# nep-pack/NonlinearEigenproblems.jl

Measured on AMD Instinct MI355X. Metric: eigenpairs/sec (gun SPMF iar m=100) + compute_Mlincomb GB/s, higher is better.
Workload: dtype f64 (complex128)

## Files before the change

nonlineareigenproblems.jl_amd/csrc/common.h:

```cpp
#pragma once
#include <hip/hip_runtime.h>
#include <stdint.h>
#include <stdio.h>
#include <stdlib.h>
#include <string.h>
#include <stdarg.h>
#include "nepmi355.h"

typedef double2 cplx;

void nep_set_error(const char* fmt, ...);

#define HIPCHK(call)                                                                       \
    do {                                                                                   \
        hipError_t e_ = (call);                                                            \
        if (e_ != hipSuccess) {                                                            \
            nep_set_error("%s:%d: %s failed: %s", __FILE__, __LINE__, #call,               \
                          hipGetErrorString(e_));                                          \
            return NEP_ERR_HIP;                                                            \
        }                                                                                  \
    } while (0)

#define ARGCHK(cond)                                                                       \
    do {                                                                                   \
// ... 104 lines not shown
extern "C" {
int nep_cw_resid_dev(nep_spmf* s, const double* d_cabs, const nep_cdouble* d_ccf, const nep_cdouble* dx, const nep_cdouble* db,
                     nep_cdouble* dr, unsigned long long* d_bits, double xsign, hipStream_t st);
int nep_mlincomb_dev_shift(nep_spmf* s, int32_t k, const nep_cdouble* dC, int64_t ldc, const nep_cdouble* dV, int64_t ldv,
                           nep_cdouble* dz, nep_cdouble* d_shift, int32_t* folded, hipStream_t st);
int32_t nep_orth_dev_mirror(const nep_cdouble* dV, int64_t ldv, int64_t rows, int32_t k, const int64_t* d_active_rows,
                            nep_cdouble* dw, nep_cdouble* d_out, int32_t method, nep_cdouble* d_mirror, int32_t nmirror,
                            nep_stream stream);
int32_t nep_orth_dev_mirror_ev(const nep_cdouble* dV, int64_t ldv, int64_t rows, int32_t k, const int64_t* d_active_rows,
                               nep_cdouble* dw, nep_cdouble* d_out, int32_t method, nep_cdouble* d_mirror, int32_t nmirror,
                               void* before_write, nep_stream stream);
int32_t nep_orth_dev_iar_next(const nep_cdouble* dV, int64_t ldv, int64_t n, int32_t k, const int64_t* d_active_rows,
                              nep_cdouble* dw, nep_cdouble* d_out, int32_t method, nep_cdouble* d_mirror, int32_t nmirror,
                              void* before_write, const nep_cdouble* dC, int64_t ldc, int32_t mt, nep_cdouble* d_WT,
                              nep_cdouble* d_shift, nep_stream stream);
int nep_spmv_wt(nep_spmf* s, const nep_cdouble* d_WT, nep_cdouble* dz, hipStream_t st);
}

struct NepTiles;
extern "C" {
int nep_tiles_build(int64_t n, int mt, int valbytes, const int32_t* rowptr, const uint32_t* idx, const void* vals, NepTiles** out);
void nep_tiles_destroy(NepTiles* t);
void nep_tiles_info(const NepTiles* t, int64_t info[8]);
size_t nep_tiles_shmem(const NepTiles* t, int k);
int nep_tiles_mlincomb(const NepTiles* t, int k, const cplx* dC, int64_t ldc, const cplx* dV, int64_t ldv, cplx* dz, cplx* d_shift,
                       hipStream_t st);
int nep_tiles_nblk(const NepTiles* t);
bool nep_tiles_resid_ok(const NepTiles* t, int k);
bool nep_tiles_resid_cm_ok(const NepTiles* t, int k);
int nep_tiles_resid_cm(const NepTiles* t, int k, const cplx* dF, const cplx* Q, int64_t ldq, cplx* R, int64_t ldr, double* partial,
// ... 21 lines not shown
```

nonlineareigenproblems.jl_amd/csrc/driver.hip:

```cpp
#include "common.h"
#include <vector>
#include <stdlib.h>
#include <time.h>

struct nep_iar {
    nep_spmf* spmf; nep_lu* lu;
    int64_t n, ldv; int32_t m, mt;
    cplx* dV; const cplx* dCtab; int64_t ldc; const int64_t* d_active;
    cplx* dz; cplx* dW;
    std::vector<double> cabs; std::vector<nep_cdouble> cf;
    cplx* dH; nep_cdouble* hH;
    double* d_cabs; cplx* d_ccf;
    cplx* hH_dev;
    int32_t method;
    std::vector<hipEvent_t> ev;
    hipStream_t side = nullptr; hipEvent_t e_solved = nullptr, e_checked = nullptr;
    hipEvent_t e_upload = nullptr; bool upload_waited = false;
    hipStream_t last = nullptr;
    bool no_events = false;
    std::vector<hipGraphExec_t> graphs;
    cplx* dWT = nullptr; int32_t wt_for = 0;
};

extern "C" {

int32_t nep_iar_create(nep_spmf* spmf, nep_lu* lu, int64_t n, int32_t m, nep_cdouble* dV, int64_t ldv,
                       const nep_cdouble* dCtab, int64_t ldc, const int64_t* d_active, nep_cdouble* dwork3n,
                       const double* h_cabs, const nep_cdouble* h_cf, int32_t mt, nep_cdouble* dH, nep_cdouble* h_pinnedH,
                       int32_t orth_method, nep_iar** out) {
    ARGCHK(out != nullptr);
    *out = nullptr;
    ARGCHK(spmf && lu && dV && dCtab && dwork3n && dH && h_pinnedH);
    ARGCHK(n > 0 && m >= 1 && ldv >= n * (int64_t)(m + 1) && ldc >= m && mt >= 1 && (orth_method == 0 || orth_method == 1));
    nep_iar* s = new nep_iar();
    s->spmf = spmf; s->lu = lu; s->n = n; s->ldv = ldv; s->m = m; s->mt = mt;
    s->dV = (cplx*)dV; s->dCtab = (const cplx*)dCtab; s->ldc = ldc; s->d_active = d_active;
    s->dz = (cplx*)dwork3n; s->dW = (cplx*)dwork3n + n;
// ... 29 lines not shown
        void* dp = nullptr;
        if (hipHostGetDevicePointer(&dp, h_pinnedH, 0) == hipSuccess) s->hH_dev = (cplx*)dp; else (void)hipGetLastError();
    }
    *out = s;
    return NEP_OK;
}

int32_t nep_iar_destroy(nep_iar* s) {
    if (!s) return NEP_OK;
    for (hipEvent_t e : s->ev) if (e) (void)hipEventDestroy(e);
    if (!s->graphs.empty()) {
        if (s->last) (void)hipStreamSynchronize(s->last);
        for (hipGraphExec_t g : s->graphs) (void)hipGraphExecDestroy(g);
    }
    if (s->side) { (void)hipStreamSynchronize(s->side); (void)hipStreamDestroy(s->side); }
    if (s->e_solved) (void)hipEventDestroy(s->e_solved);
    if (s->e_checked) (void)hipEventDestroy(s->e_checked);
    if (s->e_upload) (void)hipEventDestroy(s->e_upload);
    if (s->d_cabs) nep_pool_free_on(s->d_cabs, s->last, s->last != nullptr);
    if (s->dWT) nep_pool_free_on(s->dWT, s->last, s->last != nullptr);
    delete s;
    return NEP_OK;
}

int32_t nep_iar_step(nep_iar* s, int32_t k, int32_t refine_steps, nep_stream stream) {
    const bool skip_final = (refine_steps & 0x100) != 0 && (k % 8) != 0;
    refine_steps &= 0xff;
    ARGCHK(s && k >= 1 && k <= s->m && refine_steps >= 0 && refine_steps <= 3);
    ARGCHK(refine_steps == 0 || !s->cabs.empty());
    hipStream_t st = as_stream(stream);
    const int64_t n = s->n;
    s->last = st;
    if (s->e_upload && !s->upload_waited) { HIPCHK(hipStreamWaitEvent(st, s->e_upload, 0)); s->upload_waited = true; }
    cplx* col = s->dV + (int64_t)(k - 1) * s->ldv;
    cplx* vv = s->dV + (int64_t)k * s->ldv;
    int32_t shifted = 0;
    int rc;
    if (s->dWT && s->wt_for == k) {
        rc = nep_spmv_wt(s->spmf, (const nep_cdouble*)s->dWT, (nep_cdouble*)s->dz, st);
        shifted = 1;
    } else
        rc = nep_mlincomb_dev_shift(s->spmf, k, (const nep_cdouble*)s->dCtab, s->ldc, (const nep_cdouble*)col, n, (nep_cdouble*)s->dz,
                                    (nep_cdouble*)(vv + n), &shifted, st);
    s->wt_for = 0;
    if (rc) return rc;
    cplx* hrow = s->dH + (int64_t)(k - 1) * (s->m + 4);
    unsigned long long* bits = (unsigned long long*)(hrow + k + 2);
    const bool record = !s->cabs.empty();
    if (refine_steps == 0) {
        rc = nep_lu_solve(s->lu, 1, (const nep_cdouble*)s->dz, n, (nep_cdouble*)vv, n, -1.0, stream);
        if (rc) return rc;
    } else {
// ... 16 lines not shown
        if (s->side) {
            HIPCHK(hipEventRecord(s->e_solved, st));
            HIPCHK(hipStreamWaitEvent(s->side, s->e_solved, 0));
            cs = s->side;
        }
        rc = nep_cw_resid_dev(s->spmf, s->d_cabs, (const nep_cdouble*)s->d_ccf, (const nep_cdouble*)vv, (const nep_cdouble*)s->dz,
                              (nep_cdouble*)s->dW, bits + refine_steps, -1.0, cs);
        if (rc) return rc;
        if (s->side) { HIPCHK(hipEventRecord(s->e_checked, s->side)); before_write = (void*)s->e_checked; }
    }
    if (!shifted) {
        rc = nep_iar_shift_scale(n, k, (const nep_cdouble*)col, (nep_cdouble*)vv, stream);
        if (rc) return rc;
    }
    cplx* mirror = s->hH_dev ? s->hH_dev + (int64_t)(k - 1) * (s->m + 4) : nullptr;
    if (s->dWT && k < s->m) {
        rc = nep_orth_dev_iar_next((const nep_cdouble*)s->dV, s->ldv, n, k, s->d_active, (nep_cdouble*)vv, (nep_cdouble*)hrow, s->method,
                                   (nep_cdouble*)mirror, k + 4, before_write, (const nep_cdouble*)s->dCtab, s->ldc, s->mt,
                                   (nep_cdouble*)s->dWT, (nep_cdouble*)(vv + s->ldv + n), stream);
        if (!rc) s->wt_for = k + 1;
    } else
        rc = nep_orth_dev_mirror_ev((const nep_cdouble*)s->dV, s->ldv, n * (int64_t)(k + 1), k, s->d_active, (nep_cdouble*)vv,
                                    (nep_cdouble*)hrow, s->method, (nep_cdouble*)mirror, k + 4, before_write, stream);
    if (rc) return rc;
    if (!mirror)
        HIPCHK(hipMemcpyAsync(s->hH + (int64_t)(k - 1) * (s->m + 4), hrow, (size_t)(k + 4) * sizeof(cplx), hipMemcpyDeviceToHost, st));
    if (s->no_events) return NEP_OK;
    if (!s->ev[k]) HIPCHK(hipEventCreateWithFlags(&s->ev[k], hipEventDisableTiming | hipEventBlockingSync));
    HIPCHK(hipEventRecord(s->ev[k], st));
    return NEP_OK;
}
// ... 67 lines not shown
```

nonlineareigenproblems.jl_amd/csrc/iar_run.hip:

```cpp
#include "common.h"
#include <algorithm>
#include <deque>
#include <map>
#include <mutex>
#include <vector>
#include <math.h>
#include <time.h>

extern "C" {
int32_t nep_iar_create(nep_spmf* spmf, nep_lu* lu, int64_t n, int32_t m, nep_cdouble* dV, int64_t ldv, const nep_cdouble* dCtab,
                       int64_t ldc, const int64_t* d_active, nep_cdouble* dwork3n, const double* h_cabs, const nep_cdouble* h_cf,
                       int32_t mt, nep_cdouble* dH, nep_cdouble* h_pinnedH, int32_t orth_method, nep_iar** out);
int32_t nep_iar_steps_graph(nep_iar* s, int32_t k0, int32_t count, int32_t refine_steps, nep_stream stream, int32_t* captured);
}

namespace {

constexpr double EPS = 2.220446049250313e-16;

__global__ void k_iar_active(int64_t* act, int64_t n, int m1) {
    const int j = blockIdx.x * blockDim.x + threadIdx.x;
    if (j < m1) act[j] = (int64_t)(j + 1) * n;
}
__global__ void k_iar_start(cplx* __restrict__ V, const cplx* __restrict__ v, double inv, int64_t n) {
    const int64_t i = (int64_t)blockIdx.x * blockDim.x + threadIdx.x;
    if (i < n) V[i] = cmake(v[i].x * inv, v[i].y * inv);
}

constexpr int64_t ZSLACK = 8192;
__global__ __launch_bounds__(256) void k_iar_zero_slack(cplx* __restrict__ V, int64_t ldv, int64_t n, int m1) {
    const int j = blockIdx.y;
    const int64_t a = (int64_t)(j + 1) * n;
    const int64_t r = a + (int64_t)blockIdx.x * 256 + threadIdx.x;
    if (j < m1 && r < ldv && r < a + ZSLACK) V[(int64_t)j * ldv + r] = cmake(0.0, 0.0);
}

struct RunStreams { hipStream_t check = nullptr, eig = nullptr; hipStream_t probed_for = (hipStream_t)-1; bool shared = false; int retries = 0; };
std::mutex g_rs_mu;
std::map<int, RunStreams> g_rs;

int pick_stream(hipStream_t keep, int prio, int ncand, bool probe, const std::vector<hipStream_t>& others, hipStream_t* out, bool* shared) {
    std::vector<hipStream_t> cand;
    if (keep) cand.push_back(keep);
    hipStream_t pick = nullptr;
    for (int c = 0; c < ncand && !pick; ++c) {
        hipStream_t s = nullptr;
        if ((size_t)c < cand.size()) s = cand[c];
        else { HIPCHK(hipStreamCreateWithPriority(&s, hipStreamNonBlocking, prio)); cand.push_back(s); }
        bool clash = false;
        for (size_t i = 0; probe && i < others.size() && !clash; ++i) {
            int32_t a = 0;
            int rc = nep_stream_pair_serializes((nep_stream)others[i], (nep_stream)s, &a); if (rc) return rc;
            clash = a != 0;
        }
        if (!clash) pick = s;
    }
    if (getenv("NEP_IAR_RUN_TRACE")) fprintf(stderr, "nep_iar_run: stream pick (prio %d): %zu candidates tried, %s\n", prio, cand.size(), pick ? "free queue found" : "none free");
    if (!pick) { pick = cand[0]; *shared = true; }
    for (hipStream_t s : cand) if (s != pick) (void)hipStreamDestroy(s);
    *out = pick;
    return NEP_OK;
}

int run_streams(hipStream_t main, RunStreams* out) {
    int dev = 0; HIPCHK(hipGetDevice(&dev));
    std::lock_guard<std::mutex> lk(g_rs_mu);
    RunStreams& r = g_rs[dev];
    if (!r.check || !r.eig || r.probed_for != main || (r.shared && r.retries < 3)) {
        if (r.shared) ++r.retries;
        r.shared = false;
        int least = 0, greatest = 0;
        HIPCHK(hipDeviceGetStreamPriorityRange(&least, &greatest));
        const int ncand = getenv("NEP_IAR_EIG_CANDIDATES") ? atoi(getenv("NEP_IAR_EIG_CANDIDATES")) : 8;
        const bool probe = !(getenv("NEP_IAR_EIG_PROBE") && atoi(getenv("NEP_IAR_EIG_PROBE")) == 0);
        const int cprio = getenv("NEP_IAR_CHECK_PRIO") ? (atoi(getenv("NEP_IAR_CHECK_PRIO")) > 0 ? least : (atoi(getenv("NEP_IAR_CHECK_PRIO")) < 0 ? greatest : 0)) : 0;
        int rc = pick_stream(r.check, cprio, ncand, probe, {main}, &r.check, &r.shared); if (rc) return rc;
        const int eprio = getenv("NEP_IAR_EIG_PRIO") ? (atoi(getenv("NEP_IAR_EIG_PRIO")) < 0 ? greatest : (atoi(getenv("NEP_IAR_EIG_PRIO")) > 0 ? least : 0)) : 0;
        rc = pick_stream(r.eig, eprio, ncand, probe, {main, r.check}, &r.eig, &r.shared); if (rc) return rc;
        r.probed_for = main;
    }
    *out = r;
    return NEP_OK;
}

struct Arena {
    int dev = -1; int64_t n = 0; int32_t m = 0, mt = 0;
    cplx* Hdev = nullptr; cplx* wdev = nullptr; cplx* Ctab = nullptr; cplx* work3n = nullptr; int64_t* active = nullptr;
    cplx* v0 = nullptr; double* d_norms = nullptr; void* eigwork = nullptr; int64_t wsz = 0; int bmax = 0;
    cplx* Hpin = nullptr; cplx* wpin = nullptr; double* npin = nullptr; cplx* stage = nullptr;
    void release() {
        for (void* p : {(void*)Hdev, (void*)wdev, (void*)Ctab, (void*)work3n, (void*)active, (void*)v0, (void*)d_norms, eigwork})
            if (p) nep_pool_free(p);
        for (void* p : {(void*)Hpin, (void*)wpin, (void*)npin, (void*)stage}) if (p) (void)hipHostFree(p);
        *this = Arena();
    }
};
std::mutex g_arena_mu;
std::vector<Arena> g_arenas;
// ... 143 lines not shown
};

}

extern "C" {

int32_t nep_refine_review(int32_t umfpack_refinements, int32_t plan, int32_t final_recorded, const double* w4, int32_t hint_in,
                          int32_t out[4]) {
    ARGCHK(w4 && out && plan >= 0 && plan <= 3 && umfpack_refinements >= 0);
    Refine r; r.umf = umfpack_refinements; r.hint = hint_in;
    const bool ok = r.review(w4, plan, final_recorded != 0);
    out[0] = ok ? 1 : 0; out[1] = r.recorded; out[2] = r.hint; out[3] = r.hint_off ? 1 : 0;
    return NEP_OK;
}

int32_t nep_iar_run(nep_spmf* spmf, nep_lu* lu, int64_t n, const nep_iar_opts* opts, const nep_cdouble* h_v0,
                    const nep_cdouble* h_Ctab, int32_t mt, const double* h_cabs, const nep_cdouble* h_cf, const double* h_fro,
                    nep_fv_eval fv, void* ctx, nep_cdouble* h_lam, nep_cdouble* dQ, nep_cdouble* h_Q, double* h_err,
                    nep_cdouble* dV_basis, nep_iar_result* res, nep_stream stream) {
    ARGCHK(spmf && lu && opts && h_v0 && h_Ctab && fv && h_lam && res);
    ARGCHK(n > 0 && mt >= 1 && opts->maxit >= 1 && opts->check_error_every >= 1);
    ARGCHK(opts->orth_method == 0 || opts->orth_method == 1);
    ARGCHK(opts->errmeasure == 0 || (opts->errmeasure == 1 && h_fro));
    ARGCHK(opts->umfpack_refinements <= 0 || (h_cabs && h_cf));
    memset(res, 0, sizeof(*res));
    res->refine_plan = -1;
    struct timespec t_e_; clock_gettime(CLOCK_MONOTONIC, &t_e_);
    const double t_entry = t_e_.tv_sec * 1e3 + t_e_.tv_nsec * 1e-6;
    const int32_t m = opts->maxit;
    if (m > 128) { nep_set_error("nep_iar_run: maxit = %d exceeds the device eigen-decomposition's limit 128", m); return NEP_ERR_UNSUPPORTED; }
    const int BMAX = std::max(1, getenv("NEP_IAR_EIG_BATCH") ? atoi(getenv("NEP_IAR_EIG_BATCH")) : 16);
    const int LASTB = std::max(1, getenv("NEP_IAR_EIG_LAST") ? atoi(getenv("NEP_IAR_EIG_LAST")) : 8);
    const double T100 = getenv("NEP_IAR_EIG_MS100") ? atof(getenv("NEP_IAR_EIG_MS100")) : 3.3;
    const double TSTEP = getenv("NEP_IAR_EIG_MSSTEP") ? atof(getenv("NEP_IAR_EIG_MSSTEP")) : 0.35;
    const int cee = opts->check_error_every;
    const double neigs = opts->neigs;
    const bool unthrottled = isinf(neigs) && neigs > 0;

    Run R; R.spmf = spmf; R.lu = lu; R.n = n; R.o = *opts; R.fv = fv; R.ctx = ctx; R.h_fro = h_fro; R.st = as_stream(stream);
    R.m = m; R.mt = mt; R.ldv = n * (int64_t)(m + 1); R.h_err = h_err;
    int rc = run_streams(R.st, &R.rs); if (rc) return rc;
    rc = arena_acquire(n, m, mt, BMAX, &R.a); if (rc) return rc;
    R.have_arena = true;
    Arena& a = R.a;
    hipStream_t st = R.st, cst = R.rs.check, est = R.rs.eig;
    R.ref.umf = opts->umfpack_refinements > 0 ? opts->umfpack_refinements : 0;
    R.ref.hint = (opts->refine_hint >= 0 && !(getenv("NEP_REFINE_HINT") && atoi(getenv("NEP_REFINE_HINT")) == 0)) ? opts->refine_hint : -1;
    R.filled.assign(m + 1, 0); R.plans.assign(m + 1, 0);
    if (const char* fa = getenv("NEP_IAR_RUN_FAIL_AT")) { if (sscanf(fa, "%d:%d", &R.fail_kind, &R.fail_at) != 2) R.fail_kind = R.fail_at = 0; }
    if (h_err) for (int64_t i = 0; i < (int64_t)m * m; ++i) h_err[i] = NAN;

    if (dV_basis) { R.V = (cplx*)dV_basis; R.own_V = false; }
    else {
        void* p = nullptr;
        rc = nep_pool_alloc(&p, (size_t)(m + 1) * R.ldv * 16); if (rc) return rc;
        R.V = (cplx*)p;
// ... 10 lines not shown
    }
    hipLaunchKernelGGL(k_iar_start, dim3((unsigned)((n + 255) / 256)), dim3(256), 0, st, R.V, (const cplx*)a.v0, 1.0 / sqrt(nrm2), n);
    hipLaunchKernelGGL(k_iar_active, dim3((unsigned)((m + 1 + 63) / 64)), dim3(64), 0, st, a.active, n, m + 1);
    HIPCHK(hipMemsetAsync(a.Hdev, 0, (size_t)m * (m + 4) * 16, st));
    LAUNCHCHK();
    memset(a.Hpin, 0, (size_t)m * (m + 4) * 16);
    memset(a.wpin, 0, (size_t)m * (m + 2) * 16);
    {
        static thread_local PinnedRing ring;
        rc = ring.upload(a.Ctab, h_Ctab, (size_t)m * mt * 16, st); if (rc) return rc;
    }
    rc = nep_iar_create(spmf, lu, n, m, (nep_cdouble*)R.V, R.ldv, (const nep_cdouble*)a.Ctab, m, a.active, (nep_cdouble*)a.work3n,
                        R.ref.umf > 0 ? h_cabs : nullptr, R.ref.umf > 0 ? h_cf : nullptr, mt, (nep_cdouble*)a.Hdev,
                        (nep_cdouble*)a.Hpin, opts->orth_method, &R.step);
    if (rc) return rc;

    std::vector<char> plan_end(m + 2, 0);
    if (unthrottled) {
        std::vector<int> allk;
        for (int kk = 1; kk <= m; ++kk) if (kk % cee == 0 || kk == m) allk.push_back(kk);
        int e_ = (int)allk.size(); int size = std::min(LASTB, e_);
        while (e_ > 0) {
            plan_end[allk[e_ - 1]] = 1; e_ -= size;
            if (e_ > 0) {
                const double q = allk[e_ - 1] / 100.0;
                size = (int)std::min<double>(std::min(BMAX, e_), std::max(1.0, ceil(2.0 * T100 * q * q / (TSTEP * cee))));
            }
        }
    }
    const bool trace = getenv("NEP_IAR_RUN_TRACE") != nullptr;
    auto now = []() { struct timespec t; clock_gettime(CLOCK_MONOTONIC, &t); return t.tv_sec * 1e3 + t.tv_nsec * 1e-6; };
    double t_fv = 0;
    std::deque<int> pendA; std::deque<Batch> stA; std::deque<Check> stC;
    int slots = unthrottled ? m + 1 : std::max(BMAX, 4);
    const int CHUNK = unthrottled ? (getenv("NEP_IAR_BATCH") ? std::max(1, atoi(getenv("NEP_IAR_BATCH"))) : 8) : 4;
    const int P = std::min(256, std::max(1, 3072 / mt));
    int k = 1; bool done = false; int status = NEP_OK;
    const bool use_graph = getenv("NEP_IAR_GRAPH") && atoi(getenv("NEP_IAR_GRAPH")) != 0;
    int n_graph = 0;
    auto finished = [&]() { return R.conv >= neigs; };

    auto batch_ready = [&]() -> int {
        if (pendA.empty()) return 0;
        int cnt = 1;
        while (cnt < (int)pendA.size() && cnt < BMAX && pendA[cnt] - pendA[cnt - 1] == pendA[1] - pendA[0] && !(unthrottled && plan_end[pendA[cnt - 1]])) ++cnt;
        if (!unthrottled || plan_end[pendA[cnt - 1]] || cnt >= BMAX || done) return cnt;
        return 0;
    };
    auto launch_batch = [&](int count) -> int {
        Batch b;
        for (int i = 0; i < count; ++i) { b.kcs.push_back(pendA.front()); pendA.pop_front(); }
        const int k0 = b.kcs[0], nb = count; b.kmax = b.kcs.back();
        const int kstep = nb > 1 ? b.kcs[1] - k0 : 0;
// ... 164 lines not shown
            if (status) { drop_check(c); break; }
        }
        if (status) break;
        if (finished()) {
            done = true; pendA.clear();
            while (!stA.empty()) { drop_batch(stA.front()); stA.pop_front(); }
            while (!stC.empty()) { drop_check(stC.front()); stC.pop_front(); }
        }
        if (trace) { const double t = now(); tt_C += t - tq; tq = t; }
        if (done && pendA.empty() && stA.empty() && stC.empty()) break;
        if (!progressed) { struct timespec ts = {0, 20000}; nanosleep(&ts, nullptr); if (trace) { const double t = now(); tt_sleep += t - tq; tq = t; } }
    }
    if (trace)
        fprintf(stderr, "nep_iar_run trace (ms): set-up %.2f | loop %.2f: steps %.2f (all enqueued at %.2f) A %.2f B %.2f (callback %.2f) C %.2f sleep %.2f\n",
                t_loop - t_entry, now() - t_loop, tt_steps, t_enq_done, tt_A, tt_B, t_fv, tt_C, tt_sleep);
    if (trace && use_graph) fprintf(stderr, "nep_iar_run: %d chunks went out as hipGraphs\n", n_graph);
    if (trace && te0 && te1 && te1_rec) {
        float ms_ = 0.0f;
        if (hipEventSynchronize(te1) == hipSuccess && hipEventElapsedTime(&ms_, te0, te1) == hipSuccess)
            fprintf(stderr, "nep_iar_run: the recurrence's %d steps took %.2f ms on the device\n", m, ms_);
        (void)hipGetLastError();
    }
    if (te0) (void)hipEventDestroy(te0);
    if (te1) (void)hipEventDestroy(te1);
    while (!stA.empty()) { drop_batch(stA.front()); stA.pop_front(); }
    while (!stC.empty()) { drop_check(stC.front()); stC.pop_front(); }
    (void)hipStreamSynchronize(est);
    (void)hipStreamSynchronize(cst);
    res->retry_reason = R.retry;
    res->refine_plan = R.ref.hint_off ? -1 : (R.ref.recorded >= 0 ? R.ref.recorded : R.ref.hint);
// ... 28 lines not shown
```

nonlineareigenproblems.jl_amd/csrc/orth.hip:

```cpp
#include "common.h"
#include <vector>
#include <algorithm>
#include <math.h>
#include <stdlib.h>

typedef double orth_d2 __attribute__((ext_vector_type(2)));
template <bool NT> __device__ __forceinline__ cplx vload(const cplx* p) {
    if (NT) { const orth_d2 v = __builtin_nontemporal_load((const orth_d2*)p); return cmake(v.x, v.y); }
    return *p;
}

#define DOT_RPT 4
#define DOT_CG 8
#define DOT_RB (256 * DOT_RPT)

#define ORTH_NPART 1024
struct OrthDecide {
    const double* partial = nullptr; int np = 0; const cplx* c = nullptr; int k = 0; int method = 0; int* state = nullptr;
    cplx* out_beta = nullptr;
};
__device__ __forceinline__ void orth_pass_norms(const OrthDecide& D, double& nrm, double& p2) {
    __shared__ double smn[2][4];
    if (threadIdx.x < 256) {
        double acc = 0.0, pj = 0.0;
// ... 2 lines not shown
        acc = wave_reduce_sum(acc); pj = wave_reduce_sum(pj);
        if ((threadIdx.x & 63) == 0) { smn[0][threadIdx.x >> 6] = acc; smn[1][threadIdx.x >> 6] = pj; }
    }
    __syncthreads();
    double t = 0.0, q2 = 0.0;
    for (int q = 0; q < 4; ++q) { t += smn[0][q]; q2 += smn[1][q]; }
    __syncthreads();
    nrm = sqrt(t); p2 = q2;
}
#define ORTH_DPP_ROWS 32768
template <bool NT, bool DPP>
__global__ __launch_bounds__(256) void k_orth_dots(const cplx* __restrict__ V, int64_t ldv, int64_t rows,
                                                   int k, const int64_t* __restrict__ active,
                                                   const cplx* __restrict__ w, cplx* __restrict__ partial,
                                                   const int* __restrict__ gate = nullptr,
                                                   double* __restrict__ partial_ww = nullptr) {
    __shared__ cplx sm[DOT_CG][4];
    if (gate && *gate == 0) return;
    const int lane = threadIdx.x & 63, wv = threadIdx.x >> 6;
    const int64_t r0 = (int64_t)blockIdx.x * DOT_RB;
    cplx wr[DOT_RPT];
    int64_t rr[DOT_RPT];
#pragma unroll
    for (int i = 0; i < DOT_RPT; ++i) {
        rr[i] = r0 + threadIdx.x + 256 * i;
        wr[i] = rr[i] < rows ? w[rr[i]] : cmake(0.0, 0.0);
    }
    if (partial_ww && blockIdx.y == 0) {
        double a = 0.0;
#pragma unroll
        for (int i = 0; i < DOT_RPT; ++i) a += fma(wr[i].x, wr[i].x, wr[i].y * wr[i].y);
        a = wave_reduce_sum(a);
        if (lane == 0) sm[0][wv].x = a;
        __syncthreads();
        if (threadIdx.x == 0) partial_ww[blockIdx.x] = (sm[0][0].x + sm[0][1].x) + (sm[0][2].x + sm[0][3].x);
        __syncthreads();
    }
    int64_t rc[DOT_RPT];
#pragma unroll
    for (int i = 0; i < DOT_RPT; ++i) rc[i] = rr[i] < rows ? rr[i] : rows - 1;
    for (int j0 = blockIdx.y * DOT_CG; j0 < k; j0 += gridDim.y * DOT_CG) {
        int64_t actv[DOT_CG];
        bool grp_on = false;
#pragma unroll
        for (int jj = 0; jj < DOT_CG; ++jj) {
            const int j = j0 + jj;
            int64_t a = 0;
            if (j < k) { a = active ? active[j] : rows; if (a > rows) a = rows; }
            actv[jj] = a;
            grp_on = grp_on || r0 < a;
// ... 22 lines not shown
                    const bool on = rr[i] < actv[jj];
                    cfma_conj(acc, cmake(on ? v[jj][i].x : 0.0, on ? v[jj][i].y : 0.0), wr[i]);
                }
                accs[jj] = DPP ? wave_sum_dpp(acc) : group_reduce_sum<64>(acc);
            }
        }
#pragma unroll
        for (int jj = 0; jj < DOT_CG; ++jj)
            if (lane == 0) sm[jj][wv] = accs[jj];
        __syncthreads();
        if (threadIdx.x < DOT_CG) {
            const int j = j0 + threadIdx.x;
            if (j < k) {
                cplx t = sm[threadIdx.x][0];
                for (int q = 1; q < 4; ++q) t = cadd(t, sm[threadIdx.x][q]);
                partial[(int64_t)blockIdx.x * k + j] = t;
            }
        }
        __syncthreads();
    }
}

__global__ __launch_bounds__(256) void k_orth_reduce_h(int nb, int k, const cplx* __restrict__ partial,
                                                       cplx* __restrict__ h, const int* __restrict__ gate = nullptr,
                                                       cplx* __restrict__ hacc = nullptr, int first = 1,
                                                       int* __restrict__ state_reset = nullptr,
                                                       const OrthDecide dec = OrthDecide(), int pdone = 0,
                                                       const double* __restrict__ partial_ww = nullptr, double* __restrict__ ww = nullptr) {
    __shared__ cplx sm[4];
    if (state_reset && blockIdx.x == 0 && threadIdx.x < 16) state_reset[threadIdx.x] = 0;
    if (gate && *gate == 0) return;
// ... 279 lines not shown
    switch (nx.mt) {
        case 4: hipLaunchKernelGGL((k_orth_finish_vc<4, ROWS>), grid, block, 0, st, nx.n, kb, w, out_beta, row, mirror, nmirror, D, nx.C, nx.ldc, nx.mt, nx.WT, nx.shift_dst); break;
        case 3: hipLaunchKernelGGL((k_orth_finish_vc<3, ROWS>), grid, block, 0, st, nx.n, kb, w, out_beta, row, mirror, nmirror, D, nx.C, nx.ldc, nx.mt, nx.WT, nx.shift_dst); break;
        case 2: hipLaunchKernelGGL((k_orth_finish_vc<2, ROWS>), grid, block, 0, st, nx.n, kb, w, out_beta, row, mirror, nmirror, D, nx.C, nx.ldc, nx.mt, nx.WT, nx.shift_dst); break;
        default: hipLaunchKernelGGL((k_orth_finish_vc<1, ROWS>), grid, block, 0, st, nx.n, kb, w, out_beta, row, mirror, nmirror, D, nx.C, nx.ldc, nx.mt, nx.WT, nx.shift_dst); break;
    }
}

static int dots_grid_y(int nchunks, int k) {
    const int ngroups = (k + DOT_CG - 1) / DOT_CG;
    static int target = getenv("NEP_DOTS_TARGET") ? atoi(getenv("NEP_DOTS_TARGET")) : 6144;
    int gy = (target + nchunks - 1) / nchunks;
    return gy < 1 ? 1 : (gy > ngroups ? ngroups : gy);
}

#define ORTH_DOTS_LAUNCH(NT_, DPP_, GRID_, ST_, ...)                                                                   \
    do {                                                                                                               \
        if (NT_) { if (DPP_) hipLaunchKernelGGL((k_orth_dots<true, true>), GRID_, dim3(256), 0, ST_, __VA_ARGS__);       \
                   else hipLaunchKernelGGL((k_orth_dots<true, false>), GRID_, dim3(256), 0, ST_, __VA_ARGS__); }          \
        else { if (DPP_) hipLaunchKernelGGL((k_orth_dots<false, true>), GRID_, dim3(256), 0, ST_, __VA_ARGS__);          \
               else hipLaunchKernelGGL((k_orth_dots<false, false>), GRID_, dim3(256), 0, ST_, __VA_ARGS__); }             \
    } while (0)

static thread_local NepScratch g_orth_scratch;

static int orth_rows_k() {
    static const int v = getenv("NEP_ORTH_ROWS_K") ? atoi(getenv("NEP_ORTH_ROWS_K")) : 1 << 30;
    return v;
}

static bool orth_use_nt(int64_t rows, int64_t k, bool staircase) {
    static const int nt_env = getenv("NEP_ORTH_NT") ? atoi(getenv("NEP_ORTH_NT")) : -1;
    static const double nt_mb = getenv("NEP_ORTH_NT_MB") ? atof(getenv("NEP_ORTH_NT_MB")) : 192.0;
    static const double nt_full_mb = getenv("NEP_ORTH_NT_FULL_MB") ? atof(getenv("NEP_ORTH_NT_FULL_MB")) : 512.0;
    const double streamed_mb = 16.0e-6 * (double)rows * (double)k * (staircase ? 0.5 : 1.0);
    return nt_env >= 0 ? nt_env != 0 : streamed_mb > (staircase ? nt_mb : nt_full_mb);
}

extern "C" int32_t nep_orth(const nep_cdouble* dV, int64_t ldv, int64_t rows, int32_t k,
// ... 93 lines not shown
static int orth_dev_passes() {
    static int np = 0;
    if (!np) { const char* e = getenv("NEP_ORTH_DEV_PASSES"); np = e ? atoi(e) : 2; if (np < 1 || np > 8) np = 2; }
    return np;
}
extern "C" int32_t nep_orth_dev(const nep_cdouble* dV, int64_t ldv, int64_t rows, int32_t k,
                                const int64_t* d_active_rows, nep_cdouble* dw, nep_cdouble* d_out, int32_t method,
                                nep_stream stream) {
    return nep_orth_dev_mirror(dV, ldv, rows, k, d_active_rows, dw, d_out, method, nullptr, 0, stream);
}
extern "C" int32_t nep_orth_dev_mirror(const nep_cdouble* dV, int64_t ldv, int64_t rows, int32_t k,
                                       const int64_t* d_active_rows, nep_cdouble* dw, nep_cdouble* d_out, int32_t method,
                                       nep_cdouble* d_mirror, int32_t nmirror, nep_stream stream) {
    return nep_orth_dev_mirror_ev(dV, ldv, rows, k, d_active_rows, dw, d_out, method, d_mirror, nmirror, nullptr, stream);
}
static int orth_dev_impl(const nep_cdouble* dV, int64_t ldv, int64_t rows, int32_t k,
                         const int64_t* d_active_rows, nep_cdouble* dw, nep_cdouble* d_out, int32_t method,
                         nep_cdouble* d_mirror, int32_t nmirror, void* before_write, const OrthNextVc* next, nep_stream stream);
extern "C" int32_t nep_orth_dev_mirror_ev(const nep_cdouble* dV, int64_t ldv, int64_t rows, int32_t k,
                                          const int64_t* d_active_rows, nep_cdouble* dw, nep_cdouble* d_out, int32_t method,
                                          nep_cdouble* d_mirror, int32_t nmirror, void* before_write, nep_stream stream) {
    return orth_dev_impl(dV, ldv, rows, k, d_active_rows, dw, d_out, method, d_mirror, nmirror, before_write, nullptr, stream);
}
extern "C" int32_t nep_orth_dev_iar_next(const nep_cdouble* dV, int64_t ldv, int64_t n, int32_t k, const int64_t* d_active_rows,
                                         nep_cdouble* dw, nep_cdouble* d_out, int32_t method, nep_cdouble* d_mirror, int32_t nmirror,
                                         void* before_write, const nep_cdouble* dC, int64_t ldc, int32_t mt, nep_cdouble* d_WT,
                                         nep_cdouble* d_shift, nep_stream stream) {
    ARGCHK(dC && d_WT && d_shift && mt >= 1 && mt <= 4 && ldc >= k + 1 && n > 0);
    OrthNextVc nx; nx.C = (const cplx*)dC; nx.ldc = ldc; nx.mt = mt; nx.WT = (cplx*)d_WT; nx.shift_dst = (cplx*)d_shift; nx.n = n;
    return orth_dev_impl(dV, ldv, n * (int64_t)(k + 1), k, d_active_rows, dw, d_out, method, d_mirror, nmirror, before_write, &nx, stream);
}
static int orth_dev_impl(const nep_cdouble* dV, int64_t ldv, int64_t rows, int32_t k,
                         const int64_t* d_active_rows, nep_cdouble* dw, nep_cdouble* d_out, int32_t method,
                         nep_cdouble* d_mirror, int32_t nmirror, void* before_write, const OrthNextVc* next, nep_stream stream) {
    ARGCHK(dV && dw && d_out);
    ARGCHK(rows > 0 && k >= 1 && ldv >= rows);
    ARGCHK(method == 0 || method == 1);
    hipStream_t st = as_stream(stream);
    const int nchunks = (int)((rows + DOT_RB - 1) / DOT_RB);
    const int nblk = (int)((rows + 63) / 64);
    static const int npart_max = getenv("NEP_ORTH_NPART") ? std::max(64, atoi(getenv("NEP_ORTH_NPART"))) : ORTH_NPART;
    const int npart = std::min(nblk, npart_max);
    const int npass = method == 1 ? 1 : orth_dev_passes();
    size_t off_ph = 64;
    size_t off_c = off_ph + (size_t)nchunks * k * sizeof(cplx);
    size_t off_c2 = off_c + (size_t)k * sizeof(cplx);
    size_t off_pn = off_c2 + (size_t)k * sizeof(cplx);
    size_t off_pc2 = (off_pn + (size_t)npart * sizeof(double) + 15) & ~(size_t)15;
    size_t off_pww = off_pc2;
    size_t total = off_pww + ((size_t)nchunks + 2) * sizeof(double);
// ... 6 lines not shown
    (void)off_c2;
    double* d_pn = (double*)(base + off_pn);

    double* d_pww = (double*)(base + off_pww);
    double* d_ww = d_pww + nchunks;
    const cplx* V = (const cplx*)dV;
    cplx* w = (cplx*)dw;
    cplx* out = (cplx*)d_out;
    const size_t shm_upd = (size_t)(k + 8 * 64) * sizeof(cplx);
    const bool nt = orth_use_nt(rows, k, d_active_rows != nullptr);
    OrthDecide D;
    const bool rows_form = k <= orth_rows_k();
    const int nb_rows = (int)std::min<int64_t>((rows + 255) / 256, npart);
    D.partial = d_pn; D.np = rows_form ? nb_rows : npart; D.c = d_c; D.k = (int)k; D.method = (int)method; D.state = d_state; D.out_beta = out + k;
    {
    for (int p = 0; p < npass; ++p) {
        const int* gate = p == 0 ? nullptr : d_state + 4 + p;
        ORTH_DOTS_LAUNCH(nt, rows >= ORTH_DPP_ROWS, dim3(nchunks, dots_grid_y(nchunks, k)), st, V, ldv, rows, (int)k,
                         d_active_rows, (const cplx*)w, d_ph, gate, d_pww);
        LAUNCHCHK();
        hipLaunchKernelGGL(k_orth_reduce_h, dim3(k), dim3(256), 0, st, nchunks, (int)k, (const cplx*)d_ph, d_c, gate, out,
                           p == 0 ? 1 : 0, p == 0 ? d_state : (int*)nullptr, OrthDecide(), 0, (const double*)d_pww, d_ww);
        LAUNCHCHK();
        if (p == 0 && before_write) HIPCHK(hipStreamWaitEvent(st, (hipEvent_t)before_write, 0));
        if (rows_form) {
            const int nb = nb_rows;
            if (nt)
                hipLaunchKernelGGL(k_orth_update_rows<true>, dim3(nb), dim3(256), (size_t)k * sizeof(cplx), st, V, ldv, rows, (int)k,
                                   d_active_rows, (const cplx*)d_c, w, d_pn, gate, (const double*)d_ww, d_state, p + 1, (int)method);
            else
                hipLaunchKernelGGL(k_orth_update_rows<false>, dim3(nb), dim3(256), (size_t)k * sizeof(cplx), st, V, ldv, rows, (int)k,
                                   d_active_rows, (const cplx*)d_c, w, d_pn, gate, (const double*)d_ww, d_state, p + 1, (int)method);
        } else if (nt)
            hipLaunchKernelGGL(k_orth_update<true>, dim3(npart), dim3(512), shm_upd, st, V, ldv, rows, (int)k, d_active_rows,
                               (const cplx*)d_c, w, d_pn, gate, (const double*)d_ww, d_state, p + 1, (int)method);
// ... 68 lines not shown
```

Baseline: 1421.

## Overlap first-pass orthogonalization dots for old basis rows on a side stream

In the IAR step, the first Gram-Schmidt pass's dot products over rows beyond the first n (which don't depend on the new shifted vector's top block) are launched early on a separate stream. They run concurrently with the SpMV/solve on the main stream, and the main stream later computes only the remaining chunks and waits on an event before reducing. This is meant to hide part of the projection cost behind the linear solve. It adds stream selection (optionally with a CU mask), event synchronization and scratch reservation, and it risks contention or extra sync overhead.

```diff
diff --git a/nonlineareigenproblems.jl_amd/csrc/common.h b/nonlineareigenproblems.jl_amd/csrc/common.h
--- a/nonlineareigenproblems.jl_amd/csrc/common.h
+++ b/nonlineareigenproblems.jl_amd/csrc/common.h
@@ -142,6 +142,14 @@
                               nep_cdouble* dw, nep_cdouble* d_out, int32_t method, nep_cdouble* d_mirror, int32_t nmirror,
                               void* before_write, const nep_cdouble* dC, int64_t ldc, int32_t mt, nep_cdouble* d_WT,
                               nep_cdouble* d_shift, nep_stream stream);
+int32_t nep_orth_dev_iar_early(const nep_cdouble* dV, int64_t ldv, int64_t n, int32_t k, const int64_t* d_active_rows,
+                               const nep_cdouble* dw, int32_t method, void* side_stream, void* done_event, int32_t deps_only,
+                               int32_t* launched);
+int32_t nep_orth_dev_iar_next_late(const nep_cdouble* dV, int64_t ldv, int64_t n, int32_t k, const int64_t* d_active_rows,
+                                   nep_cdouble* dw, nep_cdouble* d_out, int32_t method, nep_cdouble* d_mirror, int32_t nmirror,
+                                   void* before_write, const nep_cdouble* dC, int64_t ldc, int32_t mt, nep_cdouble* d_WT,
+                                   nep_cdouble* d_shift, void* done_event, int32_t deps_only, nep_stream stream);
+int32_t nep_orth_dev_reserve(int64_t rows, int32_t k);
 int nep_spmv_wt(nep_spmf* s, const nep_cdouble* d_WT, nep_cdouble* dz, hipStream_t st);
 }
 
diff --git a/nonlineareigenproblems.jl_amd/csrc/driver.hip b/nonlineareigenproblems.jl_amd/csrc/driver.hip
--- a/nonlineareigenproblems.jl_amd/csrc/driver.hip
+++ b/nonlineareigenproblems.jl_amd/csrc/driver.hip
@@ -20,7 +20,10 @@
     bool no_events = false;
     std::vector<hipGraphExec_t> graphs;
     cplx* dWT = nullptr; int32_t wt_for = 0;
+    hipStream_t early = nullptr; hipEvent_t e_early = nullptr, e_fork = nullptr; int32_t early_k0 = 0; bool early_deps_only = false;
+    bool early_used = false; int32_t n_early = 0;
 };
+struct EarlyGuard { nep_iar* s; bool armed = false; ~EarlyGuard() { if (armed) (void)hipStreamSynchronize(s->early); } };
 
 extern "C" {
 
@@ -80,6 +83,9 @@
         for (hipGraphExec_t g : s->graphs) (void)hipGraphExecDestroy(g);
     }
     if (s->side) { (void)hipStreamSynchronize(s->side); (void)hipStreamDestroy(s->side); }
+    if (s->early_used) (void)hipStreamSynchronize(s->early);
+    if (s->e_early) (void)hipEventDestroy(s->e_early);
+    if (s->e_fork) (void)hipEventDestroy(s->e_fork);
     if (s->e_solved) (void)hipEventDestroy(s->e_solved);
     if (s->e_checked) (void)hipEventDestroy(s->e_checked);
     if (s->e_upload) (void)hipEventDestroy(s->e_upload);
@@ -88,6 +94,17 @@
     delete s;
     return NEP_OK;
 }
+
+int32_t nep_iar_set_early(nep_iar* s, nep_stream side, int32_t k0, int32_t deps_only) {
+    ARGCHK(s && side && k0 >= 2);
+    if (!s->dWT || s->side) return NEP_OK;
+    if (!s->e_early) HIPCHK(hipEventCreateWithFlags(&s->e_early, hipEventDisableTiming));
+    int rc = nep_orth_dev_reserve(s->n * (int64_t)(s->m + 1), s->m);
+    if (rc) return rc;
+    s->early = as_stream(side); s->early_k0 = k0; s->early_deps_only = deps_only != 0;
+    return NEP_OK;
+}
+int32_t nep_iar_early_steps(const nep_iar* s) { return s ? s->n_early : 0; }
 
 int32_t nep_iar_step(nep_iar* s, int32_t k, int32_t refine_steps, nep_stream stream) {
     const bool skip_final = (refine_steps & 0x100) != 0 && (k % 8) != 0;
@@ -102,6 +119,23 @@
     cplx* vv = s->dV + (int64_t)k * s->ldv;
     int32_t shifted = 0;
     int rc;
+    EarlyGuard early; early.s = s;
+    if (s->early && s->early_k0 >= 2 && k >= s->early_k0 && k < s->m && s->dWT && s->wt_for == k && !s->no_events && st != s->early) {
+        hipEvent_t fork = s->ev[k - 1];
+        if (!fork) {
+            if (!s->e_fork) HIPCHK(hipEventCreateWithFlags(&s->e_fork, hipEventDisableTiming));
+            HIPCHK(hipEventRecord(s->e_fork, st));
+            fork = s->e_fork;
+        }
+        HIPCHK(hipStreamWaitEvent(s->early, fork, 0));
+        int32_t launched = 0;
+        s->early_used = true; early.armed = true;
+        rc = nep_orth_dev_iar_early((const nep_cdouble*)s->dV, s->ldv, n, k, s->d_active, (const nep_cdouble*)vv, s->method,
+                                    (void*)s->early, (void*)s->e_early, s->early_deps_only ? 1 : 0, &launched);
+        if (rc) return rc;
+        early.armed = launched != 0;
+    }
+    const bool split = early.armed;
     if (s->dWT && s->wt_for == k) {
         rc = nep_spmv_wt(s->spmf, (const nep_cdouble*)s->dWT, (nep_cdouble*)s->dz, st);
         shifted = 1;
@@ -148,7 +182,13 @@
         if (rc) return rc;
     }
     cplx* mirror = s->hH_dev ? s->hH_dev + (int64_t)(k - 1) * (s->m + 4) : nullptr;
-    if (s->dWT && k < s->m) {
+    if (split) {
+        rc = nep_orth_dev_iar_next_late((const nep_cdouble*)s->dV, s->ldv, n, k, s->d_active, (nep_cdouble*)vv, (nep_cdouble*)hrow, s->method,
+                                        (nep_cdouble*)mirror, k + 4, before_write, (const nep_cdouble*)s->dCtab, s->ldc, s->mt,
+                                        (nep_cdouble*)s->dWT, (nep_cdouble*)(vv + s->ldv + n), (void*)s->e_early,
+                                        s->early_deps_only ? 1 : 0, stream);
+        if (!rc) { s->wt_for = k + 1; early.armed = false; ++s->n_early; }
+    } else if (s->dWT && k < s->m) {
         rc = nep_orth_dev_iar_next((const nep_cdouble*)s->dV, s->ldv, n, k, s->d_active, (nep_cdouble*)vv, (nep_cdouble*)hrow, s->method,
                                    (nep_cdouble*)mirror, k + 4, before_write, (const nep_cdouble*)s->dCtab, s->ldc, s->mt,
                                    (nep_cdouble*)s->dWT, (nep_cdouble*)(vv + s->ldv + n), stream);
diff --git a/nonlineareigenproblems.jl_amd/csrc/iar_run.hip b/nonlineareigenproblems.jl_amd/csrc/iar_run.hip
--- a/nonlineareigenproblems.jl_amd/csrc/iar_run.hip
+++ b/nonlineareigenproblems.jl_amd/csrc/iar_run.hip
@@ -1,5 +1,6 @@
 #include "common.h"
 #include <algorithm>
+#include <atomic>
 #include <deque>
 #include <map>
 #include <mutex>
@@ -12,6 +13,8 @@
                        int64_t ldc, const int64_t* d_active, nep_cdouble* dwork3n, const double* h_cabs, const nep_cdouble* h_cf,
                        int32_t mt, nep_cdouble* dH, nep_cdouble* h_pinnedH, int32_t orth_method, nep_iar** out);
 int32_t nep_iar_steps_graph(nep_iar* s, int32_t k0, int32_t count, int32_t refine_steps, nep_stream stream, int32_t* captured);
+int32_t nep_iar_set_early(nep_iar* s, nep_stream side, int32_t k0, int32_t deps_only);
+int32_t nep_iar_early_steps(const nep_iar* s);
 }
 
 namespace {
@@ -35,7 +38,10 @@
     if (j < m1 && r < ldv && r < a + ZSLACK) V[(int64_t)j * ldv + r] = cmake(0.0, 0.0);
 }
 
-struct RunStreams { hipStream_t check = nullptr, eig = nullptr; hipStream_t probed_for = (hipStream_t)-1; bool shared = false; int retries = 0; };
+struct RunStreams {
+    hipStream_t check = nullptr, eig = nullptr; hipStream_t probed_for = (hipStream_t)-1; bool shared = false; int retries = 0;
+    hipStream_t early = nullptr; bool early_tried = false;
+};
 std::mutex g_rs_mu;
 std::map<int, RunStreams> g_rs;
 
@@ -62,10 +68,15 @@
     return NEP_OK;
 }
 
-int run_streams(hipStream_t main, RunStreams* out) {
+int run_streams(hipStream_t main, bool want_early, RunStreams* out) {
     int dev = 0; HIPCHK(hipGetDevice(&dev));
     std::lock_guard<std::mutex> lk(g_rs_mu);
     RunStreams& r = g_rs[dev];
+    const bool repick = !r.check || !r.eig || r.probed_for != main || (r.shared && r.retries < 3);
+    if (repick && r.early_tried) {
+        if (r.early) { (void)hipStreamSynchronize(r.early); (void)hipStreamDestroy(r.early); }
+        r.early = nullptr; r.early_tried = false;
+    }
     if (!r.check || !r.eig || r.probed_for != main || (r.shared && r.retries < 3)) {
         if (r.shared) ++r.retries;
         r.shared = false;
@@ -79,9 +90,39 @@
         rc = pick_stream(r.eig, eprio, ncand, probe, {main, r.check}, &r.eig, &r.shared); if (rc) return rc;
         r.probed_for = main;
     }
+    if (want_early && !r.early_tried) {
+        r.early_tried = true;
+        if (!r.shared) {
+            const int ncand = getenv("NEP_IAR_EIG_CANDIDATES") ? atoi(getenv("NEP_IAR_EIG_CANDIDATES")) : 8;
+            hipStream_t s = nullptr; bool sh = false;
+            const int pct = getenv("NEP_IAR_EARLY_CUMASK") ? atoi(getenv("NEP_IAR_EARLY_CUMASK")) : 0;
+            if (pct > 0 && pct < 100) {
+                hipDeviceProp_t pr; HIPCHK(hipGetDeviceProperties(&pr, dev));
+                const int ncu = pr.multiProcessorCount;
+                std::vector<uint32_t> mask((ncu + 31) / 32, 0u);
+                const int period = getenv("NEP_IAR_EARLY_CUMASK_PERIOD") ? atoi(getenv("NEP_IAR_EARLY_CUMASK_PERIOD")) : 4;
+                int on = 0;
+                for (int i = 0; i < ncu; ++i) if ((i % period) * 100 < pct * period) { mask[i / 32] |= 1u << (i % 32); ++on; }
+                if (hipExtStreamCreateWithCUMask(&s, (uint32_t)mask.size(), mask.data()) != hipSuccess) { (void)hipGetLastError(); s = nullptr; }
+                if (getenv("NEP_IAR_RUN_TRACE")) fprintf(stderr, "nep_iar_run: early stream with %d of %d CUs: %s\n", on, ncu, s ? "ok" : "failed");
+                for (hipStream_t o : {main, r.check, r.eig}) {
+                    int32_t a = 0;
+                    if (s && (nep_stream_pair_serializes((nep_stream)o, (nep_stream)s, &a) != NEP_OK || a)) { (void)hipStreamDestroy(s); s = nullptr; }
+                }
+            } else
+            if (pick_stream(nullptr, 0, ncand, true, {main, r.check, r.eig}, &s, &sh) != NEP_OK) { (void)hipGetLastError(); s = nullptr; }
+            else if (sh) { (void)hipStreamDestroy(s); s = nullptr; }
+            r.early = s;
+        }
+    }
     *out = r;
+    if (!want_early) out->early = nullptr;
     return NEP_OK;
 }
+
+std::atomic<long long> g_early_steps{0};
+
+constexpr int IAR_EARLY_K0 = 2;
 
 struct Arena {
     int dev = -1; int64_t n = 0; int32_t m = 0, mt = 0;
@@ -255,6 +296,12 @@
     return NEP_OK;
 }
 
+int32_t nep_iar_early_steps_total(int64_t* out) {
+    ARGCHK(out != nullptr);
+    *out = (int64_t)g_early_steps.load();
+    return NEP_OK;
+}
+
 int32_t nep_iar_run(nep_spmf* spmf, nep_lu* lu, int64_t n, const nep_iar_opts* opts, const nep_cdouble* h_v0,
                     const nep_cdouble* h_Ctab, int32_t mt, const double* h_cabs, const nep_cdouble* h_cf, const double* h_fro,
                     nep_fv_eval fv, void* ctx, nep_cdouble* h_lam, nep_cdouble* dQ, nep_cdouble* h_Q, double* h_err,
@@ -280,7 +327,10 @@
 
     Run R; R.spmf = spmf; R.lu = lu; R.n = n; R.o = *opts; R.fv = fv; R.ctx = ctx; R.h_fro = h_fro; R.st = as_stream(stream);
     R.m = m; R.mt = mt; R.ldv = n * (int64_t)(m + 1); R.h_err = h_err;
-    int rc = run_streams(R.st, &R.rs); if (rc) return rc;
+    const bool use_graph = getenv("NEP_IAR_GRAPH") && atoi(getenv("NEP_IAR_GRAPH")) != 0;
+    const int early_mode = use_graph ? 0 : (getenv("NEP_IAR_EARLY_DOTS") ? atoi(getenv("NEP_IAR_EARLY_DOTS")) : -1);
+    int rc = run_streams(R.st, early_mode != 0, &R.rs); if (rc) return rc;
+    if (getenv("NEP_IAR_EARLY_REFUSE") && atoi(getenv("NEP_IAR_EARLY_REFUSE"))) R.rs.early = nullptr;
     rc = arena_acquire(n, m, mt, BMAX, &R.a); if (rc) return rc;
     R.have_arena = true;
     Arena& a = R.a;
@@ -321,6 +371,11 @@
                         R.ref.umf > 0 ? h_cabs : nullptr, R.ref.umf > 0 ? h_cf : nullptr, mt, (nep_cdouble*)a.Hdev,
                         (nep_cdouble*)a.Hpin, opts->orth_method, &R.step);
     if (rc) return rc;
+    if (R.rs.early) {
+        int k0 = early_mode > 0 ? 2 : IAR_EARLY_K0;
+        if (getenv("NEP_IAR_EARLY_K0")) k0 = std::max(2, atoi(getenv("NEP_IAR_EARLY_K0")));
+        rc = nep_iar_set_early(R.step, (nep_stream)R.rs.early, k0, early_mode == 2 ? 1 : 0); if (rc) return rc;
+    }
 
     std::vector<char> plan_end(m + 2, 0);
     if (unthrottled) {
@@ -343,7 +398,6 @@
     const int CHUNK = unthrottled ? (getenv("NEP_IAR_BATCH") ? std::max(1, atoi(getenv("NEP_IAR_BATCH"))) : 8) : 4;
     const int P = std::min(256, std::max(1, 3072 / mt));
     int k = 1; bool done = false; int status = NEP_OK;
-    const bool use_graph = getenv("NEP_IAR_GRAPH") && atoi(getenv("NEP_IAR_GRAPH")) != 0;
     int n_graph = 0;
     auto finished = [&]() { return R.conv >= neigs; };
 
@@ -538,6 +592,8 @@
     if (trace)
         fprintf(stderr, "nep_iar_run trace (ms): set-up %.2f | loop %.2f: steps %.2f (all enqueued at %.2f) A %.2f B %.2f (callback %.2f) C %.2f sleep %.2f\n",
                 t_loop - t_entry, now() - t_loop, tt_steps, t_enq_done, tt_A, tt_B, t_fv, tt_C, tt_sleep);
+    g_early_steps += nep_iar_early_steps(R.step);
+    if (trace) fprintf(stderr, "nep_iar_run: %d steps with the first pass' projections split over two queues\n", nep_iar_early_steps(R.step));
     if (trace && use_graph) fprintf(stderr, "nep_iar_run: %d chunks went out as hipGraphs\n", n_graph);
     if (trace && te0 && te1 && te1_rec) {
         float ms_ = 0.0f;
diff --git a/nonlineareigenproblems.jl_amd/csrc/orth.hip b/nonlineareigenproblems.jl_amd/csrc/orth.hip
--- a/nonlineareigenproblems.jl_amd/csrc/orth.hip
+++ b/nonlineareigenproblems.jl_amd/csrc/orth.hip
@@ -40,11 +40,12 @@
                                                    int k, const int64_t* __restrict__ active,
                                                    const cplx* __restrict__ w, cplx* __restrict__ partial,
                                                    const int* __restrict__ gate = nullptr,
-                                                   double* __restrict__ partial_ww = nullptr) {
+                                                   double* __restrict__ partial_ww = nullptr, int chunk0 = 0) {
     __shared__ cplx sm[DOT_CG][4];
     if (gate && *gate == 0) return;
     const int lane = threadIdx.x & 63, wv = threadIdx.x >> 6;
-    const int64_t r0 = (int64_t)blockIdx.x * DOT_RB;
+    const int chunk = blockIdx.x + chunk0;
+    const int64_t r0 = (int64_t)chunk * DOT_RB;
     cplx wr[DOT_RPT];
     int64_t rr[DOT_RPT];
 #pragma unroll
@@ -59,7 +60,7 @@
         a = wave_reduce_sum(a);
         if (lane == 0) sm[0][wv].x = a;
         __syncthreads();
-        if (threadIdx.x == 0) partial_ww[blockIdx.x] = (sm[0][0].x + sm[0][1].x) + (sm[0][2].x + sm[0][3].x);
+        if (threadIdx.x == 0) partial_ww[chunk] = (sm[0][0].x + sm[0][1].x) + (sm[0][2].x + sm[0][3].x);
         __syncthreads();
     }
     int64_t rc[DOT_RPT];
@@ -112,7 +113,7 @@
             if (j < k) {
                 cplx t = sm[threadIdx.x][0];
                 for (int q = 1; q < 4; ++q) t = cadd(t, sm[threadIdx.x][q]);
-                partial[(int64_t)blockIdx.x * k + j] = t;
+                partial[(int64_t)chunk * k + j] = t;
             }
         }
         __syncthreads();
@@ -422,15 +423,29 @@
     return gy < 1 ? 1 : (gy > ngroups ? ngroups : gy);
 }
 
-#define ORTH_DOTS_LAUNCH(NT_, DPP_, GRID_, ST_, ...)                                                                   \
+#define ORTH_DOTS_LAUNCH_LDS(NT_, DPP_, GRID_, LDS_, ST_, ...)                                                            \
     do {                                                                                                               \
-        if (NT_) { if (DPP_) hipLaunchKernelGGL((k_orth_dots<true, true>), GRID_, dim3(256), 0, ST_, __VA_ARGS__);       \
-                   else hipLaunchKernelGGL((k_orth_dots<true, false>), GRID_, dim3(256), 0, ST_, __VA_ARGS__); }          \
-        else { if (DPP_) hipLaunchKernelGGL((k_orth_dots<false, true>), GRID_, dim3(256), 0, ST_, __VA_ARGS__);          \
-               else hipLaunchKernelGGL((k_orth_dots<false, false>), GRID_, dim3(256), 0, ST_, __VA_ARGS__); }             \
+        if (NT_) { if (DPP_) hipLaunchKernelGGL((k_orth_dots<true, true>), GRID_, dim3(256), LDS_, ST_, __VA_ARGS__);    \
+                   else hipLaunchKernelGGL((k_orth_dots<true, false>), GRID_, dim3(256), LDS_, ST_, __VA_ARGS__); }       \
+        else { if (DPP_) hipLaunchKernelGGL((k_orth_dots<false, true>), GRID_, dim3(256), LDS_, ST_, __VA_ARGS__);       \
+               else hipLaunchKernelGGL((k_orth_dots<false, false>), GRID_, dim3(256), LDS_, ST_, __VA_ARGS__); }          \
     } while (0)
+#define ORTH_DOTS_LAUNCH(NT_, DPP_, GRID_, ST_, ...) ORTH_DOTS_LAUNCH_LDS(NT_, DPP_, GRID_, 0, ST_, __VA_ARGS__)
 
 static thread_local NepScratch g_orth_scratch;
+
+static size_t early_dots_lds() {
+    const size_t kb = getenv("NEP_IAR_EARLY_LDS_KB") ? (size_t)atoi(getenv("NEP_IAR_EARLY_LDS_KB")) : 0;
+    const size_t b = kb << 10;
+    if (b > 65536) {
+        (void)hipFuncSetAttribute((const void*)k_orth_dots<true, true>, hipFuncAttributeMaxDynamicSharedMemorySize, (int)b);
+        (void)hipFuncSetAttribute((const void*)k_orth_dots<true, false>, hipFuncAttributeMaxDynamicSharedMemorySize, (int)b);
+        (void)hipFuncSetAttribute((const void*)k_orth_dots<false, true>, hipFuncAttributeMaxDynamicSharedMemorySize, (int)b);
+        (void)hipFuncSetAttribute((const void*)k_orth_dots<false, false>, hipFuncAttributeMaxDynamicSharedMemorySize, (int)b);
+        (void)hipGetLastError();
+    }
+    return b;
+}
 
 static int orth_rows_k() {
     static const int v = getenv("NEP_ORTH_ROWS_K") ? atoi(getenv("NEP_ORTH_ROWS_K")) : 1 << 30;
@@ -554,9 +569,17 @@
                                        nep_cdouble* d_mirror, int32_t nmirror, nep_stream stream) {
     return nep_orth_dev_mirror_ev(dV, ldv, rows, k, d_active_rows, dw, d_out, method, d_mirror, nmirror, nullptr, stream);
 }
+static size_t orth_dev_scratch_bytes(int64_t rows, int32_t k) {
+    const size_t nchunks = (size_t)((rows + DOT_RB - 1) / DOT_RB);
+    const size_t npart = (size_t)((rows + 63) / 64);
+    const size_t off_pn = 64 + nchunks * k * sizeof(cplx) + 2 * (size_t)k * sizeof(cplx);
+    return ((off_pn + npart * sizeof(double) + 15) & ~(size_t)15) + (nchunks + 2) * sizeof(double);
+}
+struct OrthSplit { int phase = 0; int c0 = 0; hipStream_t side = nullptr; hipEvent_t done = nullptr; bool deps_only = false; };
 static int orth_dev_impl(const nep_cdouble* dV, int64_t ldv, int64_t rows, int32_t k,
                          const int64_t* d_active_rows, nep_cdouble* dw, nep_cdouble* d_out, int32_t method,
-                         nep_cdouble* d_mirror, int32_t nmirror, void* before_write, const OrthNextVc* next, nep_stream stream);
+                         nep_cdouble* d_mirror, int32_t nmirror, void* before_write, const OrthNextVc* next, nep_stream stream,
+                         const OrthSplit* split = nullptr);
 extern "C" int32_t nep_orth_dev_mirror_ev(const nep_cdouble* dV, int64_t ldv, int64_t rows, int32_t k,
                                           const int64_t* d_active_rows, nep_cdouble* dw, nep_cdouble* d_out, int32_t method,
                                           nep_cdouble* d_mirror, int32_t nmirror, void* before_write, nep_stream stream) {
@@ -570,10 +593,37 @@
     OrthNextVc nx; nx.C = (const cplx*)dC; nx.ldc = ldc; nx.mt = mt; nx.WT = (cplx*)d_WT; nx.shift_dst = (cplx*)d_shift; nx.n = n;
     return orth_dev_impl(dV, ldv, n * (int64_t)(k + 1), k, d_active_rows, dw, d_out, method, d_mirror, nmirror, before_write, &nx, stream);
 }
+extern "C" int32_t nep_orth_dev_iar_early(const nep_cdouble* dV, int64_t ldv, int64_t n, int32_t k, const int64_t* d_active_rows,
+                                          const nep_cdouble* dw, int32_t method, void* side_stream, void* done_event,
+                                          int32_t deps_only, int32_t* launched) {
+    ARGCHK(launched && side_stream && done_event && n > 0 && k >= 1);
+    *launched = 0;
+    const int64_t rows = n * (int64_t)(k + 1);
+    OrthSplit sp; sp.phase = 1; sp.c0 = (int)((n + DOT_RB - 1) / DOT_RB); sp.side = (hipStream_t)side_stream;
+    sp.done = (hipEvent_t)done_event; sp.deps_only = deps_only != 0;
+    if ((int64_t)sp.c0 >= (rows + DOT_RB - 1) / DOT_RB) return NEP_OK;
+    const int rc = orth_dev_impl(dV, ldv, rows, k, d_active_rows, (nep_cdouble*)dw, nullptr, method, nullptr, 0, nullptr, nullptr, nullptr, &sp);
+    if (!rc) *launched = 1;
+    return rc;
+}
+extern "C" int32_t nep_orth_dev_iar_next_late(const nep_cdouble* dV, int64_t ldv, int64_t n, int32_t k, const int64_t* d_active_rows,
+                                              nep_cdouble* dw, nep_cdouble* d_out, int32_t method, nep_cdouble* d_mirror, int32_t nmirror,
+                                              void* before_write, const nep_cdouble* dC, int64_t ldc, int32_t mt, nep_cdouble* d_WT,
+                                              nep_cdouble* d_shift, void* done_event, int32_t deps_only, nep_stream stream) {
+    ARGCHK(dC && d_WT && d_shift && mt >= 1 && mt <= 4 && ldc >= k + 1 && n > 0 && done_event);
+    OrthNextVc nx; nx.C = (const cplx*)dC; nx.ldc = ldc; nx.mt = mt; nx.WT = (cplx*)d_WT; nx.shift_dst = (cplx*)d_shift; nx.n = n;
+    OrthSplit sp; sp.phase = 2; sp.c0 = (int)((n + DOT_RB - 1) / DOT_RB); sp.done = (hipEvent_t)done_event; sp.deps_only = deps_only != 0;
+    return orth_dev_impl(dV, ldv, n * (int64_t)(k + 1), k, d_active_rows, dw, d_out, method, d_mirror, nmirror, before_write, &nx, stream, &sp);
+}
+extern "C" int32_t nep_orth_dev_reserve(int64_t rows, int32_t k) {
+    ARGCHK(rows > 0 && k >= 1);
+    return g_orth_scratch.ensure(orth_dev_scratch_bytes(rows, k));
+}
 static int orth_dev_impl(const nep_cdouble* dV, int64_t ldv, int64_t rows, int32_t k,
                          const int64_t* d_active_rows, nep_cdouble* dw, nep_cdouble* d_out, int32_t method,
-                         nep_cdouble* d_mirror, int32_t nmirror, void* before_write, const OrthNextVc* next, nep_stream stream) {
-    ARGCHK(dV && dw && d_out);
+                         nep_cdouble* d_mirror, int32_t nmirror, void* before_write, const OrthNextVc* next, nep_stream stream,
+                         const OrthSplit* split) {
+    ARGCHK(dV && dw && (d_out || (split && split->phase == 1)));
     ARGCHK(rows > 0 && k >= 1 && ldv >= rows);
     ARGCHK(method == 0 || method == 1);
     hipStream_t st = as_stream(stream);
@@ -610,11 +660,32 @@
     const int nb_rows = (int)std::min<int64_t>((rows + 255) / 256, npart);
     D.partial = d_pn; D.np = rows_form ? nb_rows : npart; D.c = d_c; D.k = (int)k; D.method = (int)method; D.state = d_state; D.out_beta = out + k;
     {
+    if (split && split->phase == 1) {
+        ARGCHK(split->c0 >= 1 && split->c0 < nchunks && split->side && split->done);
+        if (!split->deps_only) {
+            const int ne = nchunks - split->c0;
+            static const size_t lds = early_dots_lds();
+            ORTH_DOTS_LAUNCH_LDS(nt, rows >= ORTH_DPP_ROWS, dim3(ne, dots_grid_y(ne, k)), lds, split->side, V, ldv, rows, (int)k,
+                                 d_active_rows, (const cplx*)w, d_ph, (const int*)nullptr, d_pww, split->c0);
+            LAUNCHCHK();
+        }
+        HIPCHK(hipEventRecord(split->done, split->side));
+        return NEP_OK;
+    }
     for (int p = 0; p < npass; ++p) {
         const int* gate = p == 0 ? nullptr : d_state + 4 + p;
-        ORTH_DOTS_LAUNCH(nt, rows >= ORTH_DPP_ROWS, dim3(nchunks, dots_grid_y(nchunks, k)), st, V, ldv, rows, (int)k,
-                         d_active_rows, (const cplx*)w, d_ph, gate, d_pww);
-        LAUNCHCHK();
+        if (p == 0 && split) {
+            ARGCHK(split->phase == 2 && split->c0 >= 1 && split->c0 < nchunks && split->done);
+            const int nl = split->deps_only ? nchunks : split->c0;
+            ORTH_DOTS_LAUNCH(nt, rows >= ORTH_DPP_ROWS, dim3(nl, dots_grid_y(nl, k)), st, V, ldv, rows, (int)k,
+                             d_active_rows, (const cplx*)w, d_ph, gate, d_pww, 0);
+            LAUNCHCHK();
+            HIPCHK(hipStreamWaitEvent(st, split->done, 0));
+        } else {
+            ORTH_DOTS_LAUNCH(nt, rows >= ORTH_DPP_ROWS, dim3(nchunks, dots_grid_y(nchunks, k)), st, V, ldv, rows, (int)k,
+                             d_active_rows, (const cplx*)w, d_ph, gate, d_pww);
+            LAUNCHCHK();
+        }
         hipLaunchKernelGGL(k_orth_reduce_h, dim3(k), dim3(256), 0, st, nchunks, (int)k, (const cplx*)d_ph, d_c, gate, out,
                            p == 0 ? 1 : 0, p == 0 ? d_state : (int*)nullptr, OrthDecide(), 0, (const double*)d_pww, d_ww);
         LAUNCHCHK();
```

New measurement: 1379 (median of 2 runs). 0.971x the previous value.
